# JasperSnoek/spearmint

Hardware: NVIDIA H100
Metric: EI candidates/sec (higher is better)
Workload: dtype f32

## Files before the change

### spearmint_b200/csrc/predict_tc.cu

```cuda
#include <cuda_fp16.h>
#include <cuda.h>

#include <algorithm>
#include <vector>
#include <cstdlib>
#include <cstring>

#include "common.cuh"
#include "tc_common.cuh"

namespace smk {

__global__ void __launch_bounds__(256, 2) trtri_finalize_kernel(int Npad, int ldx, int K, const float* __restrict__ winv,
                                                                 float* X) {
  using C = Cfg<float>;
  constexpr int NB = C::NB, TM = C::TM, TN = C::TN;
  extern __shared__ __align__(16) unsigned char smem_raw[];
  TileSmem<float>& sm = *reinterpret_cast<TileSmem<float>*>(smem_raw);
  float (*Ts)[NB + kPad] = reinterpret_cast<float (*)[NB + kPad]>(smem_raw + sizeof(TileSmem<float>));
  const int nblk = Npad / NB, J = blockIdx.x, s = blockIdx.y;
  const int tid = threadIdx.x, ty = tid >> 4, tx = tid & 15;
  const float* W = winv + ((long)s * nblk + K) * NB * NB;
  float* Xt = X + (long)s * ldx * ldx + (long)K * NB * ldx + (long)J * NB;
  float acc[TM][TN];
  if (J == K) {
#pragma unroll
    for (int r = 0; r < TM; ++r)
#pragma unroll
      for (int g = 0; g < TN / 4; ++g) {
        V4<float> v = ld4(W + (long)tile_row(ty, r) * NB + g * 64 + tx * 4);
#pragma unroll
        for (int e = 0; e < 4; ++e) acc[r][g * 4 + e] = v.v[e];
      }
  } else {
#pragma unroll
    for (int r = 0; r < TM; ++r)
#pragma unroll
      for (int g = 0; g < TN / 4; ++g) {
        V4<float> v = ld4(Xt + (long)tile_row(ty, r) * ldx + g * 64 + tx * 4);
        st4(&Ts[tile_row(ty, r)][g * 64 + tx * 4], v);
      }
#pragma unroll
    for (int r = 0; r < TM; ++r)
#pragma unroll
      for (int c = 0; c < TN; ++c) acc[r][c] = 0.f;
    TileGemm<float, Lay::KContig, Lay::MContig, false>::run_bsmem(acc, W, NB, &Ts[0][0], NB + kPad, NB, sm);
  }
#pragma unroll
  for (int r = 0; r < TM; ++r)
#pragma unroll
    for (int g = 0; g < TN / 4; ++g) {
      V4<float> v;
#pragma unroll
      for (int e = 0; e < 4; ++e) v.v[e] = acc[r][g * 4 + e];
      st4(Xt + (long)tile_row(ty, r) * ldx + g * 64 + tx * 4, v);
    }
}

__global__ void __launch_bounds__(256, 2) trtri_update_kernel(int Npad, int ldx, int K, const float* __restrict__ L,
                                                               float* X) {
  using C = Cfg<float>;
  constexpr int NB = C::NB, TM = C::TM, TN = C::TN;
  __shared__ TileSmem<float> sm;
  const int I = K + 1 + blockIdx.x, J = blockIdx.y, s = blockIdx.z;
  const int tid = threadIdx.x, ty = tid >> 4, tx = tid & 15;
  const float* Lik = L + (long)s * Npad * Npad + (long)I * NB * Npad + (long)K * NB;
  float* Xs = X + (long)s * ldx * ldx;
  float* Xij = Xs + (long)I * NB * ldx + (long)J * NB;
  const float* Xkj = Xs + (long)K * NB * ldx + (long)J * NB;
  float acc[TM][TN];
  if (K == J) {
#pragma unroll
    for (int r = 0; r < TM; ++r)
#pragma unroll
      for (int c = 0; c < TN; ++c) acc[r][c] = 0.f;
  } else {
#pragma unroll
    for (int r = 0; r < TM; ++r)
#pragma unroll
      for (int g = 0; g < TN / 4; ++g) {
        V4<float> v = ld4(Xij + (long)tile_row(ty, r) * ldx + g * 64 + tx * 4);
#pragma unroll
        for (int e = 0; e < 4; ++e) acc[r][g * 4 + e] = v.v[e];
      }
  }
  TileGemm<float, Lay::KContig, Lay::MContig, true>::run(acc, Lik, Npad, Xkj, ldx, NB, sm);
#pragma unroll
  for (int r = 0; r < TM; ++r)
#pragma unroll
    for (int g = 0; g < TN / 4; ++g) {
      V4<float> v;
#pragma unroll
      for (int e = 0; e < 4; ++e) v.v[e] = acc[r][g * 4 + e];
      st4(Xij + (long)tile_row(ty, r) * ldx + g * 64 + tx * 4, v);
    }
}

__device__ __forceinline__ float tf32_hi(float x) { return tf32_rn(x); }

__global__ void split_lower_kernel(int Npad, int ld, long total, const float* __restrict__ X, float* __restrict__ hi,
                                   float* __restrict__ lo) {
  long e = (long)blockIdx.x * blockDim.x + threadIdx.x;
  if (e >= total) return;
  long per = (long)ld * ld;
  int r = (int)((e % per) / ld), c = (int)(e % ld);
  float x = (c <= r && r < Npad) ? X[e] : 0.f;
  float h = tf32_hi(x);
  hi[e] = h;
  lo[e] = x - h;
}

__global__ void __launch_bounds__(256) linv_mv_kernel(int N, int Np, const float* __restrict__ hi,
                                                      const float* __restrict__ lo, const float* __restrict__ y,
                                                      const float* __restrict__ mean, float* __restrict__ t) {
  const int s = blockIdx.y, warp = threadIdx.x >> 5, lane = threadIdx.x & 31;
  const int row = blockIdx.x * 8 + warp;
  if (row >= Np) return;
  const long base = ((long)s * Np + row) * Np;
  const float mu = mean[s];
  float acc = 0.f;
  for (int k = lane; k <= row && k < N; k += 32) acc = fmaf(hi[base + k] + lo[base + k], y[k] - mu, acc);
#pragma unroll
  for (int o = 16; o > 0; o >>= 1) acc += __shfl_xor_sync(0xffffffffu, acc, o);
  if (lane == 0) t[(long)s * Np + row] = (row < N) ? acc : 0.f;
}
__global__ void __launch_bounds__(256) linv_mtv_kernel(int N, int Np, int ld_alpha, const float* __restrict__ hi,
                                                       const float* __restrict__ lo, const float* __restrict__ t,
                                                       float* __restrict__ alpha) {
  __shared__ float red[4][64];
  const int s = blockIdx.y, cl = threadIdx.x & 63, ph = threadIdx.x >> 6;
  const int c = blockIdx.x * 64 + cl;
  const float* th = t + (long)s * Np;
  const long base = (long)s * Np * Np + c;
  float acc = 0.f;
  if (c < N)
    for (int r = (c & ~3) + ph; r < N; r += 4)
      if (r >= c) acc = fmaf(hi[base + (long)r * Np] + lo[base + (long)r * Np], th[r], acc);
  red[ph][cl] = acc;
  __syncthreads();
  if (ph == 0 && c < ld_alpha) alpha[(long)s * ld_alpha + c] = (c < N) ? red[0][cl] + red[1][cl] + red[2][cl] + red[3][cl] : 0.f;
}

__global__ void __launch_bounds__(256) linv_absmax_kernel(long per4, const float4* __restrict__ hi,
                                                          const float4* __restrict__ lo, unsigned* __restrict__ maxbits) {
  const int s = blockIdx.y;
  const float4* h = hi + (long)s * per4;
  const float4* l = lo + (long)s * per4;
  float m = 0.f;
  for (long e = (long)blockIdx.x * blockDim.x + threadIdx.x; e < per4; e += (long)gridDim.x * blockDim.x) {
    float4 a = h[e], b = l[e];
    m = fmaxf(m, fmaxf(fmaxf(fabsf(a.x + b.x), fabsf(a.y + b.y)), fmaxf(fabsf(a.z + b.z), fabsf(a.w + b.w))));
  }
#pragma unroll
  for (int o = 16; o > 0; o >>= 1) m = fmaxf(m, __shfl_xor_sync(0xffffffffu, m, o));
  if ((threadIdx.x & 31) == 0) atomicMax(&maxbits[s], __float_as_uint(m));
}

__global__ void __launch_bounds__(256) linv_pack_f16_kernel(long per4, const float4* __restrict__ hi,
                                                            const float4* __restrict__ lo,
                                                            const unsigned* __restrict__ maxbits, uint2* __restrict__ oh,
                                                            uint2* __restrict__ ol, int* __restrict__ exps) {
  const int s = blockIdx.y;
  const int eb = scale_exp(__uint_as_float(maxbits[s]));
  const float sc = ldexpf(1.f, eb);
  if (blockIdx.x == 0 && threadIdx.x == 0) exps[s] = eb;
  const long base = (long)s * per4;
  for (long e = (long)blockIdx.x * blockDim.x + threadIdx.x; e < per4; e += (long)gridDim.x * blockDim.x) {
    float4 a = hi[base + e], b = lo[base + e];
    __half hh[4], ll[4];
    split16((a.x + b.x) * sc, hh[0], ll[0]);
    split16((a.y + b.y) * sc, hh[1], ll[1]);
    split16((a.z + b.z) * sc, hh[2], ll[2]);
    split16((a.w + b.w) * sc, hh[3], ll[3]);
    oh[base + e] = pack4(hh);
    ol[base + e] = pack4(ll);
  }
}

__global__ void __launch_bounds__(256) alpha_absmax_kernel(int N, int F, int Npad_alpha, const float* __restrict__ alpha,
                                                           int* __restrict__ fexp) {
  __shared__ float red[8];
  const int s = blockIdx.x;
  float m = 0.f;
  for (long e = threadIdx.x; e < (long)F * N; e += blockDim.x) {
    int f = (int)(e / N), n = (int)(e % N);
    m = fmaxf(m, fabsf(alpha[((long)s * F + f) * Npad_alpha + n]));
  }
#pragma unroll
  for (int o = 16; o > 0; o >>= 1) m = fmaxf(m, __shfl_xor_sync(0xffffffffu, m, o));
  if ((threadIdx.x & 31) == 0) red[threadIdx.x >> 5] = m;
  __syncthreads();
  if (threadIdx.x == 0) {
    for (int w = 1; w < 8; ++w) m = fmaxf(m, red[w]);
    fexp[s] = scale_exp(m);
  }
}
__global__ void alpha_pack_f16_kernel(int N, int Np, int F, int Fp, int Npad_alpha, long total,
                                      const float* __restrict__ alpha, const int* __restrict__ fexp,
                                      __half* __restrict__ hi, __half* __restrict__ lo) {
  long e = (long)blockIdx.x * blockDim.x + threadIdx.x;
  if (e >= total) return;
  int n = (int)(e % Np);
  long sf = e / Np;
  int f = (int)(sf % Fp), s = (int)(sf / Fp);
  float x = (f < F && n < N) ? alpha[((long)s * F + f) * Npad_alpha + n] * ldexpf(1.f, fexp[s]) : 0.f;
  split16(x, hi[e], lo[e]);
}

constexpr int kKD = 16;

__global__ void __launch_bounds__(256, 2) kxt_kernel(int kind, int N, int Np, int M, int c_begin, int Mc, int D,
                                                     const float* __restrict__ X, const float* __restrict__ Cc,
                                                     const float* __restrict__ inv_ls, const float* __restrict__ amp2,
                                                     const float* __restrict__ mean, const float* __restrict__ alpha,
                                                     int Npad_alpha, __half* __restrict__ khi,
                                                     __half* __restrict__ klo, float* __restrict__ mu, int ldm) {
  constexpr int T = 128, LDC = T + kPad, LDX = T + kPad;
  __shared__ __align__(16) float cs[kKD][LDC];
  __shared__ __align__(16) float xs[kKD][LDX];
  __shared__ __align__(16) float red[16][T];
  static_assert((LDC * sizeof(float)) % 16 == 0 && (LDX * sizeof(float)) % 16 == 0, "128-bit shared loads");
  const int s = blockIdx.y, c0 = blockIdx.x * T;
  const int tid = threadIdx.x, ty = tid >> 4, tx = tid & 15;
  const float* ils = inv_ls + (long)s * D;
  const float a2 = amp2[s];
  const float2 a2s = dup2(a2 * ldexpf(1.f, kx_exp(a2)));
  const float* al = alpha ? alpha + (long)s * Npad_alpha : nullptr;
  float2 mdot[8];
#pragma unroll
  for (int r = 0; r < 8; ++r) mdot[r] = make_float2(0.f, 0.f);

  for (int n0 = 0; n0 < Np; n0 += T) {
    float2 acc[8][4];
#pragma unroll
    for (int r = 0; r < 8; ++r)
#pragma unroll
      for (int c = 0; c < 4; ++c) acc[r][c] = make_float2(0.f, 0.f);
    for (int d0 = 0; d0 < D; d0 += kKD) {
      __syncthreads();
      for (int e = tid; e < T * kKD; e += 256) {
        int row = e / kKD, dd = e % kKD, d = d0 + dd;
        int gc = min(c_begin + c0 + row, M - 1), n = n0 + row;
        float sc = (d < D) ? ils[d] : 0.f;
        cs[dd][row] = (d < D) ? Cc[(long)gc * D + d] * sc : 0.f;
        xs[dd][row] = (d < D && n < N) ? -X[(long)n * D + d] * sc : 0.f;
      }
      __syncthreads();
      const int dmax = min(kKD, D - d0);
      for (int dd = 0; dd < dmax; ++dd) {
        float2 b[4];
#pragma unroll
        for (int g = 0; g < 2; ++g) {
          const V4<float> u = ld4(&xs[dd][g * 64 + tx * 4]);
          b[2 * g] = make_float2(u.v[0], u.v[1]);
          b[2 * g + 1] = make_float2(u.v[2], u.v[3]);
        }
#pragma unroll
        for (int g = 0; g < 2; ++g) {
          const float4 p0 = *reinterpret_cast<const float4*>(&cs[dd][g * 64 + ty * 4]);
          const float2 a[4] = {dup2(p0.x), dup2(p0.y), dup2(p0.z), dup2(p0.w)};
#pragma unroll
          for (int rr = 0; rr < 4; ++rr)
#pragma unroll
            for (int c = 0; c < 4; ++c) {
              const float2 df = fadd2(a[rr], b[c]);
              acc[g * 4 + rr][c] = ffma2(df, df, acc[g * 4 + rr][c]);
            }
        }
      }
    }
    const bool edge = (n0 + T > N);
    float2 av[4];
#pragma unroll
    for (int c = 0; c < 4; ++c) {
      const int n = n0 + (c >> 1) * 64 + tx * 4 + (c & 1) * 2;
      av[c] = al ? make_float2((n < N) ? al[n] : 0.f, (n + 1 < N) ? al[n + 1] : 0.f) : make_float2(0.f, 0.f);
    }
#pragma unroll
    for (int r = 0; r < 8; ++r) {
      const long ok = ((long)s * Mc + c0 + tile_row(ty, r)) * Np + n0;
#pragma unroll
      for (int g = 0; g < 2; ++g) {
        __half2 hh[2], ll[2];
#pragma unroll
        for (int q = 0; q < 2; ++q) {
          const int c = 2 * g + q;
          float2 kk = kernel_pair_fast(kind, acc[r][c]);
          if (edge) {
            const int n = n0 + g * 64 + tx * 4 + q * 2;
            if (n >= N) kk.x = 0.f;
            if (n + 1 >= N) kk.y = 0.f;
          }
          mdot[r] = ffma2(av[c], kk, mdot[r]);
          const float2 v = fmul2(kk, a2s);
          hh[q] = __floats2half2_rn(v.x, v.y);
          const float2 hf = __half22float2(hh[q]);
          ll[q] = __floats2half2_rn(v.x - hf.x, v.y - hf.y);
        }
        uint2 ph, pl;
        ph.x = *reinterpret_cast<unsigned*>(&hh[0]); ph.y = *reinterpret_cast<unsigned*>(&hh[1]);
        pl.x = *reinterpret_cast<unsigned*>(&ll[0]); pl.y = *reinterpret_cast<unsigned*>(&ll[1]);
        *reinterpret_cast<uint2*>(khi + ok + g * 64 + tx * 4) = ph;
        *reinterpret_cast<uint2*>(klo + ok + g * 64 + tx * 4) = pl;
      }
    }
  }
  if (!al) return;
  __syncthreads();
#pragma unroll
  for (int r = 0; r < 8; ++r) red[tx][tile_row(ty, r)] = mdot[r].x + mdot[r].y;
  __syncthreads();
  if (tid < T) {
    float v = 0.f;
    for (int q = 0; q < 16; ++q) v += red[q][tid];
    int gc = c_begin + c0 + tid;
    if (gc < M) mu[(long)s * ldm + gc] = fmaf(a2, v, mean[s]);
  }
}

namespace tc {
constexpr int BM = 128;
constexpr int BN = 256;
constexpr int BK = 16;
constexpr int BK16 = 32;
constexpr int STAGES = 4;
constexpr int ROW_BYTES = BK * 4;
static_assert(ROW_BYTES == 64 && BK16 * 2 == ROW_BYTES, "operand rows must be one 64B swizzle span in both element types");
constexpr int UK_BYTES = 32;
constexpr int A_BYTES = BM * ROW_BYTES;
constexpr int B_BYTES = BN * ROW_BYTES;
constexpr int STAGE_BYTES = 2 * A_BYTES + 2 * B_BYTES;
constexpr int CONSUMERS = 2;
constexpr int THREADS = (CONSUMERS + 1) * 128;
constexpr int PRODUCER_REGS = 40, CONSUMER_REGS = 232;
static_assert(128 * PRODUCER_REGS + CONSUMERS * 128 * CONSUMER_REGS <= 65536, "register file");
constexpr int SMEM_BYTES = STAGES * STAGE_BYTES + 1024  + 256 ;

struct Args {
  int S, Np, Mc, ntiles, npairs, ngroups, ldp;
  float* partial;
  const float* z;
  float* mpartial;
  float* dbg;
  int F, M, c_begin, ldm;
  const float* mean;
  float* mu_f;
  int f16;
  int a_evict_first;
  const float* amp2;
  const int* bexp;
  int mode;
  int Npad, jb, ncols;
  float* Cmat;
  int K;
  float *xhi, *xlo, *xthi, *xtlo;
};

struct Item { int valid, rowA, rowB, k0, nk, s, tile, g, pr; };

__device__ __forceinline__ Item get_item(const Args& p, long w, int h) {
  Item it;
  it.valid = 0; it.rowA = it.rowB = it.k0 = it.nk = it.s = it.tile = it.g = it.pr = 0;
  const int bk = p.f16 ? BK16 : BK;
  if (p.mode <= 1) {
    it.pr = (int)(w % p.npairs);
    const long st = w / p.npairs;
    it.tile = (int)(st % p.ntiles);
    it.s = (int)(st / p.ntiles);
    it.g = (h == 0) ? it.pr : p.ngroups - 1 - it.pr;
    if (h == 1 && (p.mode == 1 || it.g == it.pr)) return it;
    it.nk = (p.mode == 1) ? p.Np / bk : (it.g + 1) * (BN / bk);
    it.rowA = it.s * p.Mc + it.tile * BM;
    it.rowB = (it.s * p.ngroups + it.g) * BN;
    it.valid = 1;
  } else if (p.mode == 2) {
    if (h == 1) return it;
    it.tile = (int)(w % p.ntiles);
    it.s = (int)(w / p.ntiles);
    it.rowA = it.s * p.Npad + (p.jb + it.tile) * BM;
    it.rowB = it.s * p.Npad + p.jb * BM;
    it.nk = p.jb * BM / bk;
    it.valid = 1;
  } else {
    if (h == 1) return it;
    it.tile = (int)(w % p.ntiles);
    it.s = (int)(w / p.ntiles);
    it.rowA = it.s * BM;
    it.rowB = it.s * p.Np + it.tile * BN;
    it.k0 = it.tile * BN;
    it.nk = (p.K * BM - it.tile * BN) / bk;
    it.valid = 1;
  }
  return it;
}

__global__ void __launch_bounds__(THREADS, 1)
predict_tc_kernel(const __grid_constant__ CUtensorMap mAhi, const __grid_constant__ CUtensorMap mAlo,
                  const __grid_constant__ CUtensorMap mBhi, const __grid_constant__ CUtensorMap mBlo, Args p) {
  extern __shared__ unsigned char smem_raw[];
  unsigned char* base = smem_raw + ((1024u - (smem_u32(smem_raw) & 1023u)) & 1023u);
  uint64_t* bars = reinterpret_cast<uint64_t*>(base + STAGES * STAGE_BYTES);
  uint64_t* full = bars;
  uint64_t* empty = bars + STAGES;

  const int warp = threadIdx.x >> 5, lane = threadIdx.x & 31;
  if (threadIdx.x == 0) {
    for (int i = 0; i < STAGES; ++i) { mbar_init(&full[i], 1); mbar_init(&empty[i], CONSUMERS * 4); }
    asm volatile("fence.mbarrier_init.release.cluster;" ::: "memory");
  }
  __syncthreads();

  const long nitems = (long)p.S * p.ntiles * (p.mode <= 1 ? p.npairs : 1);
  const int bk = p.f16 ? BK16 : BK;
  if (warp < 4) {
    asm volatile("setmaxnreg.dec.sync.aligned.u32 %0;" ::"n"(PRODUCER_REGS));
    if (warp == 0 && lane == 0) {
      const uint64_t hintA = (p.mode == 0 && !p.a_evict_first) ? 0x1000000000000000ull : 0x12F0000000000000ull;
      const uint64_t hintB = 0x14F0000000000000ull;
      int stage = 0;
      uint32_t phase = 0;
      for (long w = blockIdx.x; w < nitems; w += gridDim.x) {
        for (int h = 0; h < 2; ++h) {
          const Item it = get_item(p, w, h);
          if (!it.valid) break;
          for (int kc = 0; kc < it.nk; ++kc) {
            mbar_wait_relaxed(&empty[stage], phase ^ 1, 64);
            unsigned char* sb = base + stage * STAGE_BYTES;
            const int kk = it.k0 + kc * bk;
            mbar_expect_tx(&full[stage], STAGE_BYTES);
            tma_load_2d(&mAhi, &full[stage], sb, kk, it.rowA, hintA);
            tma_load_2d(&mAlo, &full[stage], sb + A_BYTES, kk, it.rowA, hintA);
            tma_load_2d(&mBhi, &full[stage], sb + 2 * A_BYTES, kk, it.rowB, hintB);
            tma_load_2d(&mBlo, &full[stage], sb + 2 * A_BYTES + B_BYTES, kk, it.rowB, hintB);
            if (++stage == STAGES) { stage = 0; phase ^= 1; }
          }
        }
      }
    }
    return;
  }

  asm volatile("setmaxnreg.inc.sync.aligned.u32 %0;" ::"n"(CONSUMER_REGS));
  const int wg = (warp >> 2) - 1;
  const int r0 = wg * 64 + (warp & 3) * 16 + (lane >> 2);
  const int cq = 2 * (lane & 3);
  const uint32_t a_off = (uint32_t)wg * 64 * ROW_BYTES;
  float d[BN / 2];
  int stage = 0;
  uint32_t phase = 0;
  for (long w = blockIdx.x; w < nitems; w += gridDim.x) {
    float acc[2] = {0.f, 0.f}, accm[2] = {0.f, 0.f};
    const Item it0 = get_item(p, w, 0);
    for (int h = 0; h < 2; ++h) {
      const Item it = get_item(p, w, h);
      if (!it.valid) break;
      int prev = -1;
      for (int kc = 0; kc < it.nk; ++kc) {
        mbar_wait(&full[stage], phase);
        const uint32_t sa = smem_u32(base + stage * STAGE_BYTES);
        const uint64_t ahi = wgmma_desc_sw64(sa + a_off), alo = wgmma_desc_sw64(sa + A_BYTES + a_off);
        const uint64_t bhi = wgmma_desc_sw64(sa + 2 * A_BYTES), blo = wgmma_desc_sw64(sa + 2 * A_BYTES + B_BYTES);
        wgmma_fence();
        if (p.f16) {
#pragma unroll
          for (int k = 0; k < ROW_BYTES / UK_BYTES; ++k) {
            const uint64_t ko = (uint64_t)((k * UK_BYTES) >> 4);
            wgmma_f16_n256(d, alo + ko, bhi + ko, (kc | k) ? 1u : 0u);
            wgmma_f16_n256(d, ahi + ko, blo + ko, 1u);
            wgmma_f16_n256(d, ahi + ko, bhi + ko, 1u);
          }
        } else {
#pragma unroll
          for (int k = 0; k < ROW_BYTES / UK_BYTES; ++k) {
            const uint64_t ko = (uint64_t)((k * UK_BYTES) >> 4);
            wgmma_tf32_n256(d, alo + ko, bhi + ko, (kc | k) ? 1u : 0u);
            wgmma_tf32_n256(d, ahi + ko, blo + ko, 1u);
            wgmma_tf32_n256(d, ahi + ko, bhi + ko, 1u);
          }
        }
        wgmma_commit();
        wgmma_wait<1>();
        if (prev >= 0 && lane == 0) mbar_arrive(&empty[prev]);
        prev = stage;
        if (++stage == STAGES) { stage = 0; phase ^= 1; }
      }
      wgmma_wait<0>();
      wgmma_hold(d);
      if (prev >= 0 && lane == 0) mbar_arrive(&empty[prev]);
      const float scl = p.f16 ? ldexpf(1.f, -(kx_exp(p.amp2[it.s]) + p.bexp[it.s])) : 1.f;
      if (p.mode == 0) {
        const float* zrow = p.z ? p.z + (long)it.s * p.Np + it.g * BN : nullptr;
#pragma unroll
        for (int nb = 0; nb < BN / 8; ++nb) {
          const int c = nb * 8 + cq;
          const float2 z2 = zrow ? __ldg(reinterpret_cast<const float2*>(zrow + c)) : make_float2(0.f, 0.f);
#pragma unroll
          for (int rh = 0; rh < 2; ++rh) {
            const float v0 = d[nb * 4 + rh * 2] * scl, v1 = d[nb * 4 + rh * 2 + 1] * scl;
            acc[rh] = fmaf(v0, v0, acc[rh]);
            acc[rh] = fmaf(v1, v1, acc[rh]);
            accm[rh] = fmaf(v0, z2.x, accm[rh]);
            accm[rh] = fmaf(v1, z2.y, accm[rh]);
            if (p.dbg) {
              float* o = p.dbg + ((long)it.s * p.Mc + it.tile * BM + r0 + 8 * rh) * p.Np + it.g * BN + c;
              o[0] = v0;
              o[1] = v1;
            }
          }
        }
      } else if (p.mode == 1) {
        const float mu0 = p.mean[it.s];
#pragma unroll
        for (int rh = 0; rh < 2; ++rh) {
          const int gc = p.c_begin + it.tile * BM + r0 + 8 * rh;
          if (gc >= p.M) continue;
#pragma unroll
          for (int nb = 0; nb < BN / 8; ++nb)
#pragma unroll
            for (int e = 0; e < 2; ++e) {
              const int f = it.g * BN + nb * 8 + cq + e;
              if (f < p.F) p.mu_f[((long)it.s * p.F + f) * p.ldm + gc] = fmaf(d[nb * 4 + rh * 2 + e], scl, mu0);
            }
        }
      } else if (p.mode == 2) {
#pragma unroll
        for (int nb = 0; nb < BN / 8; ++nb) {
          const int c = nb * 8 + cq;
          if (c >= p.ncols) continue;
#pragma unroll
          for (int rh = 0; rh < 2; ++rh) {
            float2* cp = reinterpret_cast<float2*>(
                p.Cmat + ((long)it.s * p.Npad + (long)(p.jb + it.tile) * BM + r0 + 8 * rh) * p.Npad + (long)p.jb * BM + c);
            float2 v = *cp;
            v.x -= d[nb * 4 + rh * 2];
            v.y -= d[nb * 4 + rh * 2 + 1];
            *cp = v;
          }
        }
      } else {
#pragma unroll
        for (int nb = 0; nb < BN / 8; ++nb) {
          const int jcol = it.tile * BN + nb * 8 + cq;
          if (jcol >= p.K * BM) continue;
#pragma unroll
          for (int rh = 0; rh < 2; ++rh) {
            const int row = p.K * BM + r0 + 8 * rh;
            const long xr = ((long)it.s * p.Np + row) * p.Np + jcol;
            float hh[2], ll[2];
#pragma unroll
            for (int e = 0; e < 2; ++e) {
              const float v = -d[nb * 4 + rh * 2 + e];
              hh[e] = tf32_rn(v);
              ll[e] = v - hh[e];
              const long xt = ((long)it.s * p.Np + jcol + e) * p.Np + row;
              p.xthi[xt] = hh[e];
              p.xtlo[xt] = tf32_lo(v, hh[e]);
            }
            *reinterpret_cast<float2*>(p.xhi + xr) = make_float2(hh[0], hh[1]);
            *reinterpret_cast<float2*>(p.xlo + xr) = make_float2(ll[0], ll[1]);
          }
        }
      }
    }
    if (p.mode == 0) {
#pragma unroll
      for (int rh = 0; rh < 2; ++rh) {
        float a = acc[rh], m = accm[rh];
        a += __shfl_xor_sync(0xffffffffu, a, 1);
        a += __shfl_xor_sync(0xffffffffu, a, 2);
        m += __shfl_xor_sync(0xffffffffu, m, 1);
        m += __shfl_xor_sync(0xffffffffu, m, 2);
        if ((lane & 3) == 0) {
          const long o = ((long)it0.pr * p.S + it0.s) * p.ldp + it0.tile * BM + r0 + 8 * rh;
          p.partial[o] = a;
          if (p.z) p.mpartial[o] = m;
        }
      }
    }
  }
}

__global__ void finish_var_kernel(int M, int c_begin, int Mc, int S, int npairs, int ldp, const float* __restrict__ partial,
                                  const float* __restrict__ amp2, float* __restrict__ var, int ldm, int nmp,
                                  const float* __restrict__ mu_partial, const float* __restrict__ mean,
                                  float* __restrict__ mu, const float* __restrict__ mpartial) {
  int c = blockIdx.x * blockDim.x + threadIdx.x, s = blockIdx.y;
  if (c >= Mc || c_begin + c >= M) return;
  float t = 0.f;
  for (int pr = 0; pr < npairs; ++pr) t += partial[((long)pr * S + s) * ldp + c];
  var[(long)s * ldm + c_begin + c] = amp2[s] * 1.000001f - t;
  if (mpartial) {
    float m = 0.f;
    for (int pr = 0; pr < npairs; ++pr) m += mpartial[((long)pr * S + s) * ldp + c];
    mu[(long)s * ldm + c_begin + c] = mean[s] + m;
    return;
  }
  if (nmp > 0) {
    float m = 0.f;
    for (int j = 0; j < nmp; ++j) m += mu_partial[((long)j * S + s) * ldp + c];
    mu[(long)s * ldm + c_begin + c] = fmaf(amp2[s], m, mean[s]);
  }
}

}
__global__ void kxt_mu_finish_kernel(int M, int Mc, int S, int nmp, const float* __restrict__ mu_partial,
                                     const float* __restrict__ amp2, const float* __restrict__ mean,
                                     float* __restrict__ mu, int ldm) {
  int c = blockIdx.x * blockDim.x + threadIdx.x, s = blockIdx.y;
  if (c >= M) return;
  float m = 0.f;
  for (int j = 0; j < nmp; ++j) m += mu_partial[((long)j * S + s) * Mc + c];
  mu[(long)s * ldm + c] = fmaf(amp2[s], m, mean[s]);
}
namespace tc {

typedef CUresult (*EncodeTiledFn)(CUtensorMap*, CUtensorMapDataType, cuuint32_t, void*, const cuuint64_t*,
                                  const cuuint64_t*, const cuuint32_t*, const cuuint32_t*, CUtensorMapInterleave,
                                  CUtensorMapSwizzle, CUtensorMapL2promotion, CUtensorMapFloatOOBfill);

static EncodeTiledFn encode_fn() {
  static EncodeTiledFn fn = nullptr;
  if (!fn) {
    void* p = nullptr;
    cudaDriverEntryPointQueryResult q;
    if (cudaGetDriverEntryPoint("cuTensorMapEncodeTiled", &p, cudaEnableDefault, &q) == cudaSuccess) fn = (EncodeTiledFn)p;
  }
  return fn;
}

static int make_map(CUtensorMap* m, const float* ptr, uint64_t rows, uint64_t cols, uint32_t box_rows) {
  EncodeTiledFn f = encode_fn();
  if (!f) return 1;
  cuuint64_t dims[2] = {cols, rows};
  cuuint64_t strides[1] = {cols * sizeof(float)};
  cuuint32_t box[2] = {(cuuint32_t)BK, box_rows};
  cuuint32_t estr[2] = {1, 1};
  CUresult r = f(m, CU_TENSOR_MAP_DATA_TYPE_FLOAT32, 2, const_cast<float*>(ptr), dims, strides, box, estr,
                 CU_TENSOR_MAP_INTERLEAVE_NONE, CU_TENSOR_MAP_SWIZZLE_64B, CU_TENSOR_MAP_L2_PROMOTION_L2_256B,
                 CU_TENSOR_MAP_FLOAT_OOB_FILL_NONE);
  return r == CUDA_SUCCESS ? 0 : 2;
}
static int make_map_h(CUtensorMap* m, const __half* ptr, uint64_t rows, uint64_t cols, uint32_t box_rows) {
  EncodeTiledFn f = encode_fn();
  if (!f) return 1;
  cuuint64_t dims[2] = {cols, rows};
  cuuint64_t strides[1] = {cols * sizeof(__half)};
  cuuint32_t box[2] = {(cuuint32_t)BK16, box_rows};
  cuuint32_t estr[2] = {1, 1};
  CUresult r = f(m, CU_TENSOR_MAP_DATA_TYPE_FLOAT16, 2, const_cast<__half*>(ptr), dims, strides, box, estr,
                 CU_TENSOR_MAP_INTERLEAVE_NONE, CU_TENSOR_MAP_SWIZZLE_64B, CU_TENSOR_MAP_L2_PROMOTION_L2_256B,
                 CU_TENSOR_MAP_FLOAT_OOB_FILL_NONE);
  return r == CUDA_SUCCESS ? 0 : 2;
}
}

int num_sms();
bool kxt_tc_supported(int D, int S);
bool kxt_tc_preferred(int D, int S);
int kxt_tc_ngroups(int Np);
size_t kxt_tc_workspace_bytes(int Np, int Mc, int S, int M, int D);
int kxt_tc_prepare(void* ws, int N, int Np, int M, int Mc, int D, int S, const float* X, const float* Cc, cudaStream_t st);
int kxt_tc(void* ws, int kind, int N, int Np, int M, int c_begin, int Mc, int mc_used, int D, int S, const float* inv_ls,
           const float* amp2, const float* alpha, int Npad_alpha, __half* khi, __half* klo, cudaStream_t st);
float* kxt_tc_mu_partial(void* ws, int Np, int Mc, int S, int M, int D);
static const int kKxtWsD = 32;

int tc_np(int N) { return ((N + tc::BN - 1) / tc::BN) * tc::BN; }

size_t trtri_workspace_bytes(int Np, int S) { return (size_t)S * Np * Np * sizeof(float); }

int trtri_split(int Npad, int Np, int S, const float* L, const float* winv, float* linv_hi, float* linv_lo,
                void* workspace, size_t workspace_bytes, cudaStream_t st) {
  if (Npad <= 0 || Npad % kNpadMult) return -1;
  if (Np < Npad || Np % tc::BN) return -2;
  if (S <= 0) return -3;
  if (!L || !winv || !linv_hi || !linv_lo) return -4;
  if (!workspace || workspace_bytes < trtri_workspace_bytes(Np, S)) return -8;
  float* X = reinterpret_cast<float*>(workspace);
  const size_t dsm = sizeof(TileSmem<float>) + sizeof(float) * 128 * (128 + kPad);
  static bool attr = false;
  if (!attr) {
    cudaFuncSetAttribute(trtri_finalize_kernel, cudaFuncAttributeMaxDynamicSharedMemorySize, (int)dsm);
    attr = true;
  }
  const int nblk = Npad / 128;
  timing_begin("trtri_kernel", st);
  for (int K = 0; K < nblk; ++K) {
    trtri_finalize_kernel<<<dim3(K + 1, S), 256, dsm, st>>>(Npad, Np, K, winv, X);
    if (K + 1 < nblk) trtri_update_kernel<<<dim3(nblk - K - 1, K + 1, S), 256, 0, st>>>(Npad, Np, K, L, X);
  }
  timing_end(st);
  count_launch(2 * nblk - 1);
  const long total = (long)S * Np * Np;
  split_lower_kernel<<<(unsigned)((total + 255) / 256), 256, 0, st>>>(Npad, Np, total, X, linv_hi, linv_lo);
  count_launch(1);
  return check_launch("trtri_split");
}

static void tc_args_init(tc::Args& a) {
  memset(&a, 0, sizeof(a));
}

int tc_chol_update(int Npad, int S, int jb, int ncols, float* A, const float* lhi, const float* llo, cudaStream_t st) {
  CUtensorMap mAhi, mAlo, mBhi, mBlo;
  if (tc::make_map(&mAhi, lhi, (uint64_t)S * Npad, Npad, tc::BM) || tc::make_map(&mAlo, llo, (uint64_t)S * Npad, Npad, tc::BM) ||
      tc::make_map(&mBhi, lhi, (uint64_t)S * Npad, Npad, tc::BN) || tc::make_map(&mBlo, llo, (uint64_t)S * Npad, Npad, tc::BN))
    return 1999;
  static bool attr = false;
  if (!attr) {
    cudaFuncSetAttribute(tc::predict_tc_kernel, cudaFuncAttributeMaxDynamicSharedMemorySize, tc::SMEM_BYTES);
    attr = true;
  }
  tc::Args a;
  tc_args_init(a);
  a.mode = 2; a.S = S; a.Npad = Npad; a.jb = jb; a.ncols = ncols; a.Cmat = A;
  a.ntiles = Npad / tc::BM - jb; a.npairs = 1; a.ngroups = 1;
  long nitems = (long)S * a.ntiles;
  int grid = (int)std::min<long>(nitems, num_sms());
  timing_begin("tc_chol_update", st);
  tc::predict_tc_kernel<<<grid, tc::THREADS, tc::SMEM_BYTES, st>>>(mAhi, mAlo, mBhi, mBlo, a);
  timing_end(st);
  count_launch();
  return check_launch("tc_chol_update");
}

__global__ void __launch_bounds__(256, 2) trtri_lt_kernel(int Npad, int K, const float* __restrict__ L,
                                                           const float* __restrict__ winv, float* __restrict__ lthi,
                                                           float* __restrict__ ltlo) {
  using C = Cfg<float>;
  constexpr int NB = C::NB, TM = C::TM, TN = C::TN;
  __shared__ TileSmem<float> sm;
  const int nblk = Npad / NB, J = blockIdx.x, s = blockIdx.y;
  const int tid = threadIdx.x, ty = tid >> 4, tx = tid & 15;
  const float* W = winv + ((long)s * nblk + K) * NB * NB;
  const float* Lk = L + (long)s * Npad * Npad + (long)K * NB * Npad + (long)J * NB;
  float acc[TM][TN];
#pragma unroll
  for (int r = 0; r < TM; ++r)
#pragma unroll
    for (int c = 0; c < TN; ++c) acc[r][c] = 0.f;
  TileGemm<float, Lay::KContig, Lay::MContig, false>::run(acc, W, NB, Lk, Npad, NB, sm);
  const long off = (long)s * NB * Npad + (long)J * NB;
#pragma unroll
  for (int r = 0; r < TM; ++r)
#pragma unroll
    for (int g = 0; g < TN / 4; ++g) {
      V4<float> h, l;
#pragma unroll
      for (int e = 0; e < 4; ++e) {
        float x = acc[r][g * 4 + e];
        h.v[e] = tf32_hi(x);
        l.v[e] = tf32_lo(x, h.v[e]);
      }
      const long o = off + (long)tile_row(ty, r) * Npad + g * 64 + tx * 4;
      st4(lthi + o, h);
      st4(ltlo + o, l);
    }
}

__global__ void trtri_diag_store_kernel(int Npad, int Np, int K, const float* __restrict__ winv, float* __restrict__ xhi,
                                        float* __restrict__ xlo, float* __restrict__ xthi, float* __restrict__ xtlo) {
  constexpr int NB = 128;
  const int s = blockIdx.y, nblk = Npad / NB;
  const float* W = winv + ((long)s * nblk + K) * NB * NB;
  for (int e = blockIdx.x * blockDim.x + threadIdx.x; e < NB * NB; e += gridDim.x * blockDim.x) {
    int i = e / NB, k = e % NB;
    float x = W[e], h = tf32_hi(x), l = x - h;
    long o = ((long)s * Np + (long)K * NB + i) * Np + (long)K * NB + k;
    long ot = ((long)s * Np + (long)K * NB + k) * Np + (long)K * NB + i;
    xhi[o] = h; xlo[o] = l; xthi[ot] = h; xtlo[ot] = tf32_lo(x, h);
  }
}

size_t trtri_tc_workspace_bytes(int Npad, int Np, int S) {
  return (2 * (size_t)S * Np * Np + 2 * (size_t)S * 128 * Npad) * sizeof(float);
}

int potrf_lower_batched_tc(int, int, float*, float*, int*, float*, float*, cudaStream_t, cudaEvent_t*);
void potrf_winv_block(int, int, int, const float*, float*, cudaStream_t);

static int trtri_tc_run(int Npad, int Np, int S, const float* L, float* winv, float* linv_hi, float* linv_lo,
                        void* workspace, size_t workspace_bytes, cudaStream_t st, cudaEvent_t* blk_done) {
  if (Npad <= 0 || Npad % kNpadMult) return -1;
  if (Np < Npad || Np % tc::BN) return -2;
  if (S <= 0) return -3;
  if (!L || !winv || !linv_hi || !linv_lo) return -4;
  if (!workspace || workspace_bytes < trtri_tc_workspace_bytes(Npad, Np, S)) return -8;
  float* xthi = reinterpret_cast<float*>(workspace);
  float* xtlo = xthi + (size_t)S * Np * Np;
  float* lthi = xtlo + (size_t)S * Np * Np;
  float* ltlo = lthi + (size_t)S * 128 * Npad;
  const size_t xb = (size_t)S * Np * Np * sizeof(float);
  cudaMemsetAsync(linv_hi, 0, xb, st);
  cudaMemsetAsync(linv_lo, 0, xb, st);
  cudaMemsetAsync(xthi, 0, 2 * xb, st);
  CUtensorMap mAhi, mAlo, mBhi, mBlo;
  if (tc::make_map(&mAhi, lthi, (uint64_t)S * 128, Npad, tc::BM) || tc::make_map(&mAlo, ltlo, (uint64_t)S * 128, Npad, tc::BM) ||
      tc::make_map(&mBhi, xthi, (uint64_t)S * Np, Np, tc::BN) || tc::make_map(&mBlo, xtlo, (uint64_t)S * Np, Np, tc::BN))
    return 1999;
  static bool attr = false;
  if (!attr) {
    cudaFuncSetAttribute(tc::predict_tc_kernel, cudaFuncAttributeMaxDynamicSharedMemorySize, tc::SMEM_BYTES);
    attr = true;
  }
  const int nblk = Npad / 128;
  timing_begin("trtri_kernel", st);
  for (int K = 0; K < nblk; ++K) {
    if (blk_done) {
      cudaStreamWaitEvent(st, blk_done[K], 0);
      potrf_winv_block(Npad, S, K, L, winv, st);
    }
    trtri_diag_store_kernel<<<dim3(8, S), 256, 0, st>>>(Npad, Np, K, winv, linv_hi, linv_lo, xthi, xtlo);
    count_launch();
    if (K == 0) continue;
    trtri_lt_kernel<<<dim3(K, S), 256, 0, st>>>(Npad, K, L, winv, lthi, ltlo);
    tc::Args a;
    tc_args_init(a);
    a.mode = 3; a.S = S; a.Np = Np; a.Npad = Npad; a.K = K;
    a.ntiles = (K * 128 + tc::BN - 1) / tc::BN; a.npairs = 1; a.ngroups = 1;
    a.xhi = linv_hi; a.xlo = linv_lo; a.xthi = xthi; a.xtlo = xtlo;
    long nitems = (long)S * a.ntiles;
    int grid = (int)std::min<long>(nitems, num_sms());
    tc::predict_tc_kernel<<<grid, tc::THREADS, tc::SMEM_BYTES, st>>>(mAhi, mAlo, mBhi, mBlo, a);
    count_launch(2);
  }
  timing_end(st);
  return check_launch("trtri_split_tc");
}

int trtri_split_tc(int Npad, int Np, int S, const float* L, const float* winv, float* linv_hi, float* linv_lo,
                   void* workspace, size_t workspace_bytes, cudaStream_t st) {
  return trtri_tc_run(Npad, Np, S, L, const_cast<float*>(winv), linv_hi, linv_lo, workspace, workspace_bytes, st, nullptr);
}

int potrf_trtri_tc(int Npad, int Np, int S, float* A, float* winv, int* info, float* lhi, float* llo, float* linv_hi,
                   float* linv_lo, void* tws, size_t tws_bytes, cudaStream_t st) {
  if (Npad <= 0 || Npad % kNpadMult) return -1;
  static cudaStream_t aux = nullptr;
  static cudaEvent_t ev_in = nullptr, ev_out = nullptr;
  static std::vector<cudaEvent_t> blk;
  if (!aux) {
    cudaStreamCreateWithFlags(&aux, cudaStreamNonBlocking);
    cudaEventCreateWithFlags(&ev_in, cudaEventDisableTiming);
    cudaEventCreateWithFlags(&ev_out, cudaEventDisableTiming);
  }
  const int nblk = Npad / 128;
  while ((int)blk.size() < nblk) {
    cudaEvent_t e;
    cudaEventCreateWithFlags(&e, cudaEventDisableTiming);
    blk.push_back(e);
  }
  cudaEventRecord(ev_in, st);
  cudaStreamWaitEvent(aux, ev_in, 0);
  int rc = potrf_lower_batched_tc(Npad, S, A, winv, info, lhi, llo, st, blk.data());
  if (rc) return rc;
  rc = trtri_tc_run(Npad, Np, S, A, winv, linv_hi, linv_lo, tws, tws_bytes, aux, blk.data());
  cudaEventRecord(ev_out, aux);
  cudaStreamWaitEvent(st, ev_out, 0);
  return rc;
}

int linv_pack_f16(int Np, int S, const float* linv_hi, const float* linv_lo, __half* out_hi, __half* out_lo, int* exps,
                  cudaStream_t st) {
  if (Np <= 0 || Np % tc::BN) return -1;
  if (S <= 0) return -2;
  if (!linv_hi || !linv_lo || !out_hi || !out_lo || !exps) return -3;
  unsigned* maxbits = reinterpret_cast<unsigned*>(exps + S);
  cudaMemsetAsync(maxbits, 0, sizeof(unsigned) * S, st);
  const long per4 = (long)Np * Np / 4;
  const int gx = (int)std::min<long>((per4 + 255) / 256, 4L * num_sms());
  timing_begin("linv_pack_f16", st);
  linv_absmax_kernel<<<dim3(gx, S), 256, 0, st>>>(per4, reinterpret_cast<const float4*>(linv_hi),
                                                  reinterpret_cast<const float4*>(linv_lo), maxbits);
  linv_pack_f16_kernel<<<dim3(gx, S), 256, 0, st>>>(per4, reinterpret_cast<const float4*>(linv_hi),
                                                    reinterpret_cast<const float4*>(linv_lo), maxbits,
                                                    reinterpret_cast<uint2*>(out_hi), reinterpret_cast<uint2*>(out_lo), exps);
  timing_end(st);
  count_launch(2);
  return check_launch("linv_pack_f16");
}

int linv_alpha(int N, int Np, int S, const float* linv_hi, const float* linv_lo, const float* y, const float* mean,
               float* alpha, int ld_alpha, float* tmp, cudaStream_t st) {
  if (N <= 0 || Np < N) return -1;
  if (S <= 0) return -3;
  if (!linv_hi || !linv_lo || !y || !mean || !alpha || !tmp) return -4;
  if (ld_alpha < N) return -9;
  linv_mv_kernel<<<dim3((Np + 7) / 8, S), 256, 0, st>>>(N, Np, linv_hi, linv_lo, y, mean, tmp);
  linv_mtv_kernel<<<dim3((ld_alpha + 63) / 64, S), 256, 0, st>>>(N, Np, ld_alpha, linv_hi, linv_lo, tmp, alpha);
  count_launch(2);
  return check_launch("linv_alpha");
}

static bool tc_overlap_enabled() {
  static int v = -1;
  if (v < 0) { const char* e = getenv("SMK_TC_OVERLAP"); v = (e && e[0] == '1') ? 1 : 0; }
  return v == 1;
}
static size_t tc_chunk_cands(int Np, int M, int S, size_t budget) {
  size_t per_cand = (size_t)S * Np * 2 * sizeof(__half);
  size_t mpad = ((size_t)M + 127) / 128 * 128;
  size_t mc = budget / per_cand;
  if (mc >= mpad) return mpad;
  if (tc_overlap_enabled()) mc = (budget / 2) / per_cand;
  mc = mc / 128 * 128;
  if (mc < 128) mc = 128;
  return mc;
}
static int tc_nbuf(int Np, int M, int S, size_t budget) {
  size_t mpad = ((size_t)M + 127) / 128 * 128;
  if (!tc_overlap_enabled()) return 1;
  return tc_chunk_cands(Np, M, S, budget) >= mpad ? 1 : 2;
}
static size_t tc_budget() {
  const char* e = getenv("SMK_TC_BUDGET_MB");
  if (e && e[0]) { long mb = atol(e); if (mb > 0) return (size_t)mb << 20; }
  return (size_t)20 << 30;
}
#define kTcBudget (tc_budget())

static int fant_rows(int F) { return F > 1 ? ((F + tc::BN - 1) / tc::BN) * tc::BN : 0; }

size_t predict_tc_workspace_bytes(int Np, int M, int S, int F) {
  size_t mc = tc_chunk_cands(Np, M, S, kTcBudget);
  int ngroups = Np / tc::BN, npairs = (ngroups + 1) / 2, nbuf = tc_nbuf(Np, M, S, kTcBudget);
  return (size_t)nbuf * S * mc * Np * 2 * sizeof(__half) + 2 * (size_t)npairs * S * mc * sizeof(float) +
         2 * (size_t)S * fant_rows(F) * Np * sizeof(__half) + (size_t)S * sizeof(int) + 1024 +
         kxt_tc_workspace_bytes(Np, (int)mc, S, M, kKxtWsD);
}

size_t kxt_pack_workspace_bytes(int Np, int M, int S) {
  return kxt_tc_workspace_bytes(Np, ((M + 127) / 128) * 128, S, M, kKxtWsD) + 256;
}
int kxt_pack(int impl, int kind, int N, int Np, int M, int D, int S, const float* X, const float* Cc, const float* inv_ls,
             const float* amp2, const float* mean, const float* alpha, int Npad_alpha, __half* khi, __half* klo,
             float* mu, int ldm, void* workspace, size_t workspace_bytes, cudaStream_t st) {
  if (kind < 0 || kind > 3) return -2;
  if (N <= 0 || Np < N || Np % tc::BN) return -4;
  if (M <= 0 || D <= 0 || S <= 0) return -5;
  if (!X || !Cc || !inv_ls || !amp2 || !mean || !alpha || !khi || !klo || !mu) return -8;
  if (ldm < M) return -18;
  const int Mc = ((M + 127) / 128) * 128;
  if (impl == 0) {
    kxt_kernel<<<dim3(Mc / 128, S), 256, 0, st>>>(kind, N, Np, M, 0, Mc, D, X, Cc, inv_ls, amp2, mean, alpha, Npad_alpha,
                                                  khi, klo, mu, ldm);
    count_launch();
    return check_launch("kxt_pack");
  }
  if (!kxt_tc_supported(D, S)) return -1;
  if (!workspace || workspace_bytes < kxt_pack_workspace_bytes(Np, M, S)) return -20;
  const int nmp = kxt_tc_ngroups(Np);
  int rc = kxt_tc_prepare(workspace, N, Np, M, Mc, D, S, X, Cc, st);
  if (rc) return rc;
  rc = kxt_tc(workspace, kind, N, Np, M, 0, Mc, Mc, D, S, inv_ls, amp2, alpha, Npad_alpha, khi, klo, st);
  if (rc) return rc;
  float* mu_partial = kxt_tc_mu_partial(workspace, Np, Mc, S, M, D);
  kxt_mu_finish_kernel<<<dim3((Mc + 255) / 256, S), 256, 0, st>>>(M, Mc, S, nmp, mu_partial, amp2, mean, mu, ldm);
  count_launch();
  return check_launch("kxt_pack");
}

struct PregenState {
  bool valid = false;
  void* ws = nullptr;
  int M = 0, S = 0, Np = 0, N = 0;
  cudaEvent_t done = nullptr, fork = nullptr;
  cudaStream_t stream = nullptr;
};
static PregenState g_pregen;

int predict_tc_pregen(int kind, int N, int Np, int M, int D, int S, const float* X, const float* Cc, const float* inv_ls,
                      const float* amp2, void* workspace, size_t workspace_bytes, int F, cudaStream_t st) {
  if (kind < 0 || kind > 3) return -1;
  if (N <= 0 || Np < N || Np % tc::BN) return -3;
  if (M <= 0 || D <= 0 || S <= 0) return -4;
  if (!X || !Cc || !inv_ls || !amp2) return -7;
  const bool fant = F > 1;
  if (!workspace || workspace_bytes < predict_tc_workspace_bytes(Np, M, S, fant ? F : 1)) return -20;
  if (tc_nbuf(Np, M, S, kTcBudget) != 1) return -22;
  const int Mc = (int)tc_chunk_cands(Np, M, S, kTcBudget);
  const int ngroups = Np / tc::BN, npairs = (ngroups + 1) / 2;
  const size_t kelems = (size_t)S * Mc * Np;
  __half* kbase = reinterpret_cast<__half*>(workspace);
  float* partial = reinterpret_cast<float*>(kbase + 2 * kelems);
  const int Fp = fant ? fant_rows(F) : 0;
  __half* ahi = reinterpret_cast<__half*>(partial + 2 * (size_t)npairs * S * Mc);
  int* fexp = reinterpret_cast<int*>(ahi + 2 * (size_t)S * Fp * Np);
  void* kws = reinterpret_cast<void*>(fexp + S);
  static int gen_env = -1;
  if (gen_env < 0) { const char* e = getenv("SMK_KXT_IMPL"); gen_env = (e && !strcmp(e, "tc")) ? 1 : 0; }
  const bool gen_tc = gen_env == 1 && kxt_tc_preferred(D, S);
  PregenState& g = g_pregen;
  if (!g.stream) {
    cudaStreamCreateWithFlags(&g.stream, cudaStreamNonBlocking);
    cudaEventCreateWithFlags(&g.done, cudaEventDisableTiming);
    cudaEventCreateWithFlags(&g.fork, cudaEventDisableTiming);
  }
  cudaEventRecord(g.fork, st);
  cudaStreamWaitEvent(g.stream, g.fork, 0);
  const int mc_used = min(Mc, (M + 127) / 128 * 128);
  timing_begin("kxt_kernel", g.stream);
  if (gen_tc) {
    int rc = kxt_tc_prepare(kws, N, Np, M, Mc, D, S, X, Cc, g.stream);
    if (rc) return rc;
    rc = kxt_tc(kws, kind, N, Np, M, 0, Mc, mc_used, D, S, inv_ls, amp2, nullptr, 0, kbase, kbase + kelems, g.stream);
    if (rc) return rc;
  } else {
    kxt_kernel<<<dim3(mc_used / 128, S), 256, 0, g.stream>>>(kind, N, Np, M, 0, Mc, D, X, Cc, inv_ls, amp2, nullptr, nullptr, 0,
                                                             kbase, kbase + kelems, nullptr, 0);
    count_launch();
  }
  timing_end(g.stream);
  cudaEventRecord(g.done, g.stream);
  g.valid = true; g.ws = workspace; g.M = M; g.S = S; g.Np = Np; g.N = N;
  return check_launch("predict_tc_pregen");
}

int predict_tc(int kind, int N, int Np, int M, int D, int S, const float* X, const float* Cc, const float* inv_ls,
               const float* amp2, const float* mean, const __half* linv_hi, const __half* linv_lo, const int* linv_exp,
               const float* alpha, int Npad_alpha, float* mu, float* var, int ldm, void* workspace,
               size_t workspace_bytes, float* dbg, int F, const float* alpha_f, float* mu_f, const float* z,
               int pregenerated, cudaStream_t st) {
  if (kind < 0 || kind > 3) return -1;
  if (N <= 0) return -2;
  if (Np < N || Np % tc::BN) return -3;
  if (M <= 0) return -4;
  if (D <= 0) return -5;
  if (S <= 0) return -6;
  if (!X || !Cc || !inv_ls || !amp2 || !mean || !linv_hi || !linv_lo || !linv_exp || !alpha || !mu || !var) return -7;
  if (ldm < M) return -19;
  const bool fant = (F > 1 && alpha_f && mu_f);
  if (!workspace || workspace_bytes < predict_tc_workspace_bytes(Np, M, S, fant ? F : 1)) return -20;
  const int Mc = (int)tc_chunk_cands(Np, M, S, kTcBudget);
  const int nbuf = tc_nbuf(Np, M, S, kTcBudget);
  const int ngroups = Np / tc::BN, npairs = (ngroups + 1) / 2;
  const size_t kelems = (size_t)S * Mc * Np;
  __half* kbase = reinterpret_cast<__half*>(workspace);
  float* partial = reinterpret_cast<float*>(kbase + (size_t)nbuf * 2 * kelems);
  float* mpartial = partial + (size_t)npairs * S * Mc;
  const int Fp = fant ? fant_rows(F) : 0;
  __half* ahi = reinterpret_cast<__half*>(mpartial + (size_t)npairs * S * Mc);
  __half* alo = ahi + (size_t)S * Fp * Np;
  int* fexp = reinterpret_cast<int*>(alo + (size_t)S * Fp * Np);
  static int gen_env = -1;
  if (gen_env < 0) { const char* e = getenv("SMK_KXT_IMPL"); gen_env = (e && !strcmp(e, "tc")) ? 1 : 0; }
  const bool gen_tc = gen_env == 1 && kxt_tc_preferred(D, S) && nbuf == 1;
  const int nmp = (gen_tc && !z) ? kxt_tc_ngroups(Np) : 0;
  void* kws = reinterpret_cast<void*>(fexp + S);
  float* mu_partial = gen_tc ? kxt_tc_mu_partial(kws, Np, Mc, S, M, D) : nullptr;
  const float* gen_alpha = z ? nullptr : alpha;
  const bool pre = pregenerated && z && nbuf == 1 && g_pregen.valid && g_pregen.ws == workspace && g_pregen.M == M &&
                   g_pregen.S == S && g_pregen.Np == Np && g_pregen.N == N;
  if (pregenerated && !pre) return -21;
  if (g_pregen.valid && g_pregen.ws == workspace) {
    cudaStreamWaitEvent(st, g_pregen.done, 0);
    g_pregen.valid = false;
  }
  if (!pre && gen_tc) {
    int rc = kxt_tc_prepare(kws, N, Np, M, Mc, D, S, X, Cc, st);
    if (rc) return rc;
  }
  CUtensorMap mFhi, mFlo;
  if (fant) {
    const long total = (long)S * Fp * Np;
    alpha_absmax_kernel<<<S, 256, 0, st>>>(N, F, Npad_alpha, alpha_f, fexp);
    alpha_pack_f16_kernel<<<(unsigned)((total + 255) / 256), 256, 0, st>>>(N, Np, F, Fp, Npad_alpha, total, alpha_f, fexp,
                                                                           ahi, alo);
    count_launch(2);
    if (tc::make_map_h(&mFhi, ahi, (uint64_t)S * Fp, Np, tc::BN) || tc::make_map_h(&mFlo, alo, (uint64_t)S * Fp, Np, tc::BN))
      return 1999;
  }

  CUtensorMap mAhi[2], mAlo[2], mBhi, mBlo;
  for (int b = 0; b < nbuf; ++b) {
    __half* kh = kbase + (size_t)b * 2 * kelems;
    if (tc::make_map_h(&mAhi[b], kh, (uint64_t)S * Mc, Np, tc::BM) ||
        tc::make_map_h(&mAlo[b], kh + kelems, (uint64_t)S * Mc, Np, tc::BM))
      return 1999;
  }
  if (tc::make_map_h(&mBhi, linv_hi, (uint64_t)S * Np, Np, tc::BN) || tc::make_map_h(&mBlo, linv_lo, (uint64_t)S * Np, Np, tc::BN))
    return 1999;
  static bool attr = false;
  if (!attr) {
    cudaFuncSetAttribute(tc::predict_tc_kernel, cudaFuncAttributeMaxDynamicSharedMemorySize, tc::SMEM_BYTES);
    attr = true;
  }
  static cudaStream_t aux = nullptr;
  static cudaEvent_t ev_fork = nullptr, ev_kxt[2] = {nullptr, nullptr}, ev_mma[2] = {nullptr, nullptr};
  if (!aux) {
    cudaStreamCreateWithFlags(&aux, cudaStreamNonBlocking);
    cudaEventCreateWithFlags(&ev_fork, cudaEventDisableTiming);
    for (int i = 0; i < 2; ++i) {
      cudaEventCreateWithFlags(&ev_kxt[i], cudaEventDisableTiming);
      cudaEventCreateWithFlags(&ev_mma[i], cudaEventDisableTiming);
    }
  }
  const bool overlap = (nbuf == 2);
  cudaStream_t kst = overlap ? aux : st;
  if (overlap) {
    cudaEventRecord(ev_fork, st);
    cudaStreamWaitEvent(aux, ev_fork, 0);
  }
  int ci = 0;
  for (int c_begin = 0; c_begin < M; c_begin += Mc, ++ci) {
    const int b = overlap ? (ci & 1) : 0;
    __half* kh = kbase + (size_t)b * 2 * kelems;
    const int mc_used = min(Mc, ((M - c_begin) + 127) / 128 * 128);
    if (overlap && ci >= 2) cudaStreamWaitEvent(aux, ev_mma[b], 0);
    if (!(pre && ci == 0)) {
      timing_begin("kxt_kernel", kst);
      if (gen_tc) {
        int rc = kxt_tc(kws, kind, N, Np, M, c_begin, Mc, mc_used, D, S, inv_ls, amp2, gen_alpha, Npad_alpha, kh, kh + kelems, kst);
        if (rc) return rc;
      } else {
        kxt_kernel<<<dim3(mc_used / 128, S), 256, 0, kst>>>(kind, N, Np, M, c_begin, Mc, D, X, Cc, inv_ls, amp2, mean,
                                                            gen_alpha, Npad_alpha, kh, kh + kelems, mu, ldm);
      }
      timing_end(kst);
    }
    if (overlap) {
      cudaEventRecord(ev_kxt[b], aux);
      cudaStreamWaitEvent(st, ev_kxt[b], 0);
    }
    tc::Args a;
    tc_args_init(a);
    a.S = S; a.Np = Np; a.Mc = Mc; a.ntiles = mc_used / tc::BM; a.npairs = npairs; a.ngroups = ngroups; a.ldp = Mc;
    a.partial = partial; a.dbg = dbg; a.z = z; a.mpartial = mpartial;
    a.M = M; a.c_begin = c_begin; a.ldm = ldm; a.mean = mean;
    a.mode = 0; a.f16 = 1; a.amp2 = amp2; a.bexp = linv_exp;
    { const char* e = getenv("SMK_TC_A_EVICT_FIRST"); a.a_evict_first = (e && e[0] == '1') ? 1 : 0; }
    long nitems = (long)S * a.ntiles * npairs;
    int grid = (int)std::min<long>(nitems, num_sms());
    timing_begin("predict_tc_kernel", st);
    tc::predict_tc_kernel<<<grid, tc::THREADS, tc::SMEM_BYTES, st>>>(mAhi[b], mAlo[b], mBhi, mBlo, a);
    timing_end(st);
    tc::finish_var_kernel<<<dim3((mc_used + 255) / 256, S), 256, 0, st>>>(M, c_begin, mc_used, S, npairs, Mc, partial,
                                                                        amp2, var, ldm, nmp, mu_partial, mean, mu,
                                                                        z ? mpartial : nullptr);
    count_launch(3);
    if (fant) {
      tc::Args r = a;
      r.mode = 1; r.F = F; r.mu_f = mu_f; r.bexp = fexp; r.z = nullptr; r.ngroups = Fp / tc::BN; r.npairs = r.ngroups;
      long nit = (long)S * r.ntiles * r.npairs;
      int gr = (int)std::min<long>(nit, num_sms());
      timing_begin("predict_tc_kernel_rect", st);
      tc::predict_tc_kernel<<<gr, tc::THREADS, tc::SMEM_BYTES, st>>>(mAhi[b], mAlo[b], mFhi, mFlo, r);
      timing_end(st);
      count_launch();
    }
    if (overlap) cudaEventRecord(ev_mma[b], st);
  }
  return check_launch("predict_tc");
}

}
```

Baseline: 207,500.

## Fuse trtri diagonal store into L^T kernel and zero only needed regions

Folds the diagonal-block hi/lo store into the trtri_lt_kernel as extra blocks, which removes one kernel launch per block step. The transposed store is now staged through shared memory so writes are coalesced instead of strided. The three full-buffer memsets are replaced by one custom zero kernel that clears only the regions the later kernels do not overwrite. This cuts memset bandwidth and launch count, but correctness now depends on the zero pattern exactly covering every unwritten area, notably the odd-kb rule for the transposed buffers.

```diff
diff --git a/spearmint_b200/csrc/predict_tc.cu b/spearmint_b200/csrc/predict_tc.cu
--- a/spearmint_b200/csrc/predict_tc.cu
+++ b/spearmint_b200/csrc/predict_tc.cu
@@ -724,15 +724,46 @@
   return check_launch("tc_chol_update");
 }
 
-__global__ void __launch_bounds__(256, 2) trtri_lt_kernel(int Npad, int K, const float* __restrict__ L,
+constexpr int kDiagRows = 32;
+__device__ __forceinline__ void trtri_diag_store(int Np, int K, int r0, const float* __restrict__ W, float* __restrict__ xhi,
+                                                 float* __restrict__ xlo, float* __restrict__ xthi, float* __restrict__ xtlo,
+                                                 float (*T)[129], long sbase) {
+  constexpr int NB = 128, R = kDiagRows;
+  for (int e = threadIdx.x; e < R * NB; e += blockDim.x) {
+    const int i = e / NB, k = e % NB;
+    const float x = W[(long)(r0 + i) * NB + k], h = tf32_hi(x);
+    const long o = (sbase + (long)K * NB + r0 + i) * Np + (long)K * NB + k;
+    xhi[o] = h;
+    xlo[o] = x - h;
+    T[i][k] = x;
+  }
+  __syncthreads();
+  for (int e = threadIdx.x; e < R * NB; e += blockDim.x) {
+    const int k = e / R, i = e % R;
+    const float x = T[i][k], h = tf32_hi(x);
+    const long ot = (sbase + (long)K * NB + k) * Np + (long)K * NB + r0 + i;
+    xthi[ot] = h;
+    xtlo[ot] = tf32_lo(x, h);
+  }
+}
+
+__global__ void __launch_bounds__(256, 2) trtri_lt_kernel(int Npad, int Np, int K, const float* __restrict__ L,
                                                            const float* __restrict__ winv, float* __restrict__ lthi,
-                                                           float* __restrict__ ltlo) {
+                                                           float* __restrict__ ltlo, float* __restrict__ xhi,
+                                                           float* __restrict__ xlo, float* __restrict__ xthi,
+                                                           float* __restrict__ xtlo) {
   using C = Cfg<float>;
   constexpr int NB = C::NB, TM = C::TM, TN = C::TN;
   __shared__ TileSmem<float> sm;
+  static_assert(sizeof(TileSmem<float>) >= kDiagRows * 129 * sizeof(float), "diagonal-store staging fits the GEMM tiles");
   const int nblk = Npad / NB, J = blockIdx.x, s = blockIdx.y;
   const int tid = threadIdx.x, ty = tid >> 4, tx = tid & 15;
   const float* W = winv + ((long)s * nblk + K) * NB * NB;
+  if (J >= K) {
+    trtri_diag_store(Np, K, (J - K) * kDiagRows, W, xhi, xlo, xthi, xtlo, reinterpret_cast<float (*)[129]>(&sm),
+                     (long)s * Np);
+    return;
+  }
   const float* Lk = L + (long)s * Npad * Npad + (long)K * NB * Npad + (long)J * NB;
   float acc[TM][TN];
 #pragma unroll
@@ -758,17 +789,21 @@
     }
 }
 
-__global__ void trtri_diag_store_kernel(int Npad, int Np, int K, const float* __restrict__ winv, float* __restrict__ xhi,
-                                        float* __restrict__ xlo, float* __restrict__ xthi, float* __restrict__ xtlo) {
-  constexpr int NB = 128;
-  const int s = blockIdx.y, nblk = Npad / NB;
-  const float* W = winv + ((long)s * nblk + K) * NB * NB;
-  for (int e = blockIdx.x * blockDim.x + threadIdx.x; e < NB * NB; e += gridDim.x * blockDim.x) {
-    int i = e / NB, k = e % NB;
-    float x = W[e], h = tf32_hi(x), l = x - h;
-    long o = ((long)s * Np + (long)K * NB + i) * Np + (long)K * NB + k;
-    long ot = ((long)s * Np + (long)K * NB + k) * Np + (long)K * NB + i;
-    xhi[o] = h; xlo[o] = l; xthi[ot] = h; xtlo[ot] = tf32_lo(x, h);
+__global__ void __launch_bounds__(256) trtri_zero_kernel(int Npad, int Np, float* __restrict__ xhi, float* __restrict__ xlo,
+                                                         float* __restrict__ xthi, float* __restrict__ xtlo) {
+  const int r = blockIdx.x * 8 + (threadIdx.x >> 5), lane = threadIdx.x & 31;
+  if (r >= Np) return;
+  const long row = ((long)blockIdx.y * Np + r) * Np;
+  const float4 z = make_float4(0.f, 0.f, 0.f, 0.f);
+  const int kb = r / 128;
+  for (int c = (r < Npad ? (kb + 1) * 128 : 0) + lane * 4; c < Np; c += 128) {
+    *reinterpret_cast<float4*>(xhi + row + c) = z;
+    *reinterpret_cast<float4*>(xlo + row + c) = z;
+  }
+  if (r < Npad && (kb & 1)) {
+    const int c = (kb - 1) * 128 + lane * 4;
+    *reinterpret_cast<float4*>(xthi + row + c) = z;
+    *reinterpret_cast<float4*>(xtlo + row + c) = z;
   }
 }
 
@@ -790,10 +825,8 @@
   float* xtlo = xthi + (size_t)S * Np * Np;
   float* lthi = xtlo + (size_t)S * Np * Np;
   float* ltlo = lthi + (size_t)S * 128 * Npad;
-  const size_t xb = (size_t)S * Np * Np * sizeof(float);
-  cudaMemsetAsync(linv_hi, 0, xb, st);
-  cudaMemsetAsync(linv_lo, 0, xb, st);
-  cudaMemsetAsync(xthi, 0, 2 * xb, st);
+  trtri_zero_kernel<<<dim3(Np / 8, S), 256, 0, st>>>(Npad, Np, linv_hi, linv_lo, xthi, xtlo);
+  count_launch();
   CUtensorMap mAhi, mAlo, mBhi, mBlo;
   if (tc::make_map(&mAhi, lthi, (uint64_t)S * 128, Npad, tc::BM) || tc::make_map(&mAlo, ltlo, (uint64_t)S * 128, Npad, tc::BM) ||
       tc::make_map(&mBhi, xthi, (uint64_t)S * Np, Np, tc::BN) || tc::make_map(&mBlo, xtlo, (uint64_t)S * Np, Np, tc::BN))
@@ -810,10 +843,9 @@
       cudaStreamWaitEvent(st, blk_done[K], 0);
       potrf_winv_block(Npad, S, K, L, winv, st);
     }
-    trtri_diag_store_kernel<<<dim3(8, S), 256, 0, st>>>(Npad, Np, K, winv, linv_hi, linv_lo, xthi, xtlo);
+    trtri_lt_kernel<<<dim3(K + 128 / kDiagRows, S), 256, 0, st>>>(Npad, Np, K, L, winv, lthi, ltlo, linv_hi, linv_lo, xthi, xtlo);
     count_launch();
     if (K == 0) continue;
-    trtri_lt_kernel<<<dim3(K, S), 256, 0, st>>>(Npad, K, L, winv, lthi, ltlo);
     tc::Args a;
     tc_args_init(a);
     a.mode = 3; a.S = S; a.Np = Np; a.Npad = Npad; a.K = K;
@@ -822,7 +854,7 @@
     long nitems = (long)S * a.ntiles;
     int grid = (int)std::min<long>(nitems, num_sms());
     tc::predict_tc_kernel<<<grid, tc::THREADS, tc::SMEM_BYTES, st>>>(mAhi, mAlo, mBhi, mBlo, a);
-    count_launch(2);
+    count_launch();
   }
   timing_end(st);
   return check_launch("trtri_split_tc");
```

After: 208,400 (median of 6 runs). Within noise of the previous version (+0.5%).
